# aexoden/snesimage

Hardware: AMD Instinct MI355X
Metric: candidate palettes scored/sec (higher is better)
Workload: dtype f32

## Files before the change

### snesimage_amd/csrc/capi.hip

```cpp
#include "../../include/snesimage_hip.h"
#include "kernels.hpp"
#include "kernels_opt.hpp"
#include "kernels_fast.hpp"
#include "kernels_sparse.hpp"
#include "kernels_sparse2.hpp"
#include "kernels_batch.hpp"
#include "kernels_shared.hpp"
#include "kernels_tile.hpp"
#include "kernels_level.hpp"
#include "kernels_char.hpp"
#include "kernels_char_set.hpp"
#include "kernels_guide.hpp"
#include "kernels_guide_lab.hpp"
#include "kernels_guide_window.hpp"

#include <hip/hip_runtime.h>

#include <atomic>
#include <cmath>
#include <cstdio>
#include <cstdlib>
#include <cstring>
#include <string>
#include <utility>
// ... 124 lines not shown
        bool counters_cleared = false;
        uint32_t h2q_max = 512;
        bool down_tiles = true;
        uint32_t h0_min = 1024;
        bool base_down_side = false;
        uint32_t h0_grid = 8192;
        hipStream_t h0_stream[8] = {}; hipEvent_t ev_scan[8] = {}, ev_h0[8] = {}, ev_hn[8] = {}, ev_vn[8] = {};
        bool v0_aside = true;
        hipEvent_t ev_v0[8] = {};
        bool vn_aside = true;
        uint32_t tiles_grid = 4096;
        uint32_t down1_grid = 32768;
        bool vsplit = true;
        uint32_t scan4_max = 2048;
        uint32_t hgrid = 8192;
        bool dedup = true; uint32_t dedup_min = 1024; int *holder = nullptr; bool holder_dirty = false;
        bool enabled = false, side = true; uint32_t min_n = 1; uint32_t cap = 0, lanes = 0;
        SparseGeom S{};
        float *store = nullptr, *cand_tab = nullptr, *cand_lab = nullptr, *ckf = nullptr, *ckh = nullptr; long long zeros_off = 0; uint32_t *bitmap = nullptr; double *cka = nullptr, *part = nullptr;
        CandMeta *meta = nullptr; unsigned int *items = nullptr; int *item_count = nullptr; long long item_stride = 0; int *order = nullptr, *first = nullptr;
        uint4 *plist = nullptr; int *plist_count = nullptr; bool plist_valid = false;
        hipStream_t base_stream = nullptr; hipEvent_t ev_base_in = nullptr, ev_base_h = nullptr, ev_base_done = nullptr, ev_base_narrow = nullptr;
        uint8_t *dmaps = nullptr, *dmapsC4 = nullptr;
        uint8_t *bmap = nullptr, *bmapC4 = nullptr, *bcand = nullptr; unsigned long long *dpack = nullptr; double *ckd = nullptr; uint32_t slot_ci = 0;
        float *rec_lab = nullptr;
        int base_sp = -1, base_si = -1;
        struct Ahead { uint8_t *bmap = nullptr, *bmapC4 = nullptr, *bcand = nullptr; unsigned long long *dpack = nullptr; double *ckd = nullptr; float *btab = nullptr, *blab = nullptr, *rec_lab = nullptr; int *ok = nullptr;
                       hipEvent_t ev = nullptr; bool on = true, have = false; int sp = -1, si = -1; unsigned long long epoch = 0; } ahead;
    } sp;
    uint8_t *d_cand = nullptr; uint32_t cand_cap = 0;
// ... 361 lines not shown
    return SNES_OK;
}

SparseParams sparse_params(snesimage_ctx *c, uint32_t lane) {
    auto &sp = c->sp;
    SparseParams P{};
    P.G = c->G; P.S = sp.S; P.K = c->K; P.ncol = c->ncol; P.base = (int)(sp.lanes * sp.cap);
    P.pack = c->d_pack; P.packC4 = c->d_packC4; P.packR4 = c->d_packR4; P.plist = sp.plist; P.plist_count = sp.plist_count;
    P.pal_lin = c->d_pal_lin; P.pal_xyb = c->d_pal_xyb; P.cand_tab = sp.cand_tab;
    P.perceptual = c->perceptual ? 1 : 0; P.labpx = c->d_labpx_t; P.cand_lab = sp.cand_lab; P.bitmap = sp.bitmap;
    P.img1C4 = c->d_img1C4; P.mu1R4 = c->d_mu1R4; P.sd1R4 = c->d_sd1R4; P.a1R4 = c->d_a1R4; P.r1R4 = c->d_r1R4;
    P.store = sp.store; P.meta = sp.meta;
    P.items = sp.items + (size_t)lane * sp.item_stride * kItemLists; P.item_count = sp.item_count + (size_t)lane * kItemLists; P.item_stride = sp.item_stride;
    P.ckf = sp.ckf; P.cka = sp.cka; P.part = sp.part; P.first = sp.first; P.ckh = sp.ckh; P.zeros = sp.ckh + sp.zeros_off; P.trash = sp.ckh + sp.zeros_off + 12LL * c->G.W;
    for (P.s_first = 0; P.s_first < c->G.nscales && c->G.sw[P.s_first] >= 64; P.s_first++) {}
    if (c->dither) {
        const uint32_t l = lane < c->nlanes ? lane : 0;
        P.use_maps = 1; P.sub_size = (int)c->sub_size; P.slot_ci = sp.slot_ci; P.subC4 = c->d_subC4; P.tile_pal = c->d_tile_pal;
        P.perceptual = 0; P.labpx = sp.rec_lab;
        P.maps = sp.dmaps + (size_t)l * sp.cap * c->npx; P.mapsC4 = sp.dmapsC4 + (size_t)l * sp.cap * c->npx; P.bmap = sp.bmap; P.bmapC4 = sp.bmapC4;
    }
    return P;
}

static size_t h2_lds(const snesimage_ctx *c) { return sizeof(float) * 3 * (size_t)(c->ncol + 2); }

int32_t sparse_base_pass(snesimage_ctx *c, int sp_idx, int si, uint32_t n_cand) {
    auto &sp = c->sp;
    const Geom &G = c->G;
    if (!sp.plist_valid) {
// ... 474 lines not shown
    if (const char *e = getenv("SNES_DITHER_REC")) c->dither_rec = atoi(e) != 0;
    if (const char *e = getenv("SNES_DITHER4_MAX")) { int v = atoi(e); if (v >= 0) c->dither4_max = (uint32_t)v; }
    if (const char *e = getenv("SNES_DOWN1_GRID")) { int v = atoi(e); if (v >= 64) c->sp.down1_grid = (uint32_t)v; }
    if (const char *e = getenv("SNES_VSPLIT")) c->sp.vsplit = atoi(e) != 0;
    if (const char *e = getenv("SNES_DOWN_TILES")) c->sp.down_tiles = atoi(e) != 0;
    if (const char *e = getenv("SNES_V0_ASIDE")) c->sp.v0_aside = atoi(e) != 0;
    if (const char *e = getenv("SNES_VN_ASIDE")) c->sp.vn_aside = atoi(e) != 0;
    if (const char *e = getenv("SNES_H0_GRID")) { int v = atoi(e); if (v >= 16) c->sp.h0_grid = (uint32_t)v; }
    if (const char *e = getenv("SNES_H0_MIN")) { int v = atoi(e); if (v >= 0) c->sp.h0_min = (uint32_t)v; }
    if (const char *e = getenv("SNES_TILES_GRID")) { int v = atoi(e); if (v >= 64) c->sp.tiles_grid = (uint32_t)v; }
    if (const char *e = getenv("SNES_SCAN4_MAX")) { int v = atoi(e); if (v >= 0) c->sp.scan4_max = (uint32_t)v; }
    if (const char *e = getenv("SNES_H2Q_MAX")) { int v = atoi(e); if (v >= 0) c->sp.h2q_max = (uint32_t)v; }
    if (const char *e = getenv("SNES_HGRID")) { int v = atoi(e); if (v >= 1) c->sp.hgrid = (uint32_t)v; }
    if (const char *e = getenv("SNES_SPARSE_MIN")) { int v = atoi(e); if (v >= 1) c->sp.min_n = (uint32_t)v; }
    if (const char *e = getenv("SNES_DEDUP")) c->sp.dedup = atoi(e) != 0;
    if (const char *e = getenv("SNES_DEDUP_MIN")) { int v = atoi(e); if (v >= 1) c->sp.dedup_min = (uint32_t)v; }
    Geom &G = c->G;
    G.W = (int)w; G.H = (int)h; G.nscales = 0;
    int P2 = 8;
    while (P2 < (int)h) P2 *= 2;
    for (int s = 0; s < kMaxScales; s++) {
        if (s > 0 && (G.sw[s - 1] < 8 || G.th[s - 1] < 8)) break;
        G.sw[s] = (int)w >> s; G.th[s] = s == 0 ? (int)h : (G.th[s - 1] + 1) / 2; G.sh[s] = s == 0 ? (int)h : P2 >> s; G.nscales = s + 1;
    }
    long long off = 0, soff = 0;
    for (int s = 0; s < G.nscales; s++) {
        long long N = (long long)G.sw[s] * G.sh[s];
        G.src_off[s] = soff; soff += 3 * N;
        if (s >= 1) { G.off_xyb[s] = off; off += 3 * N; G.off_xybT[s] = off; off += 3 * N; } else { G.off_xyb[s] = 0; G.off_xybT[s] = 0; }
        G.off_hout[s] = off; off += 9 * N;
// ... 553 lines not shown
```

### snesimage_amd/csrc/kernels.hpp

```cpp
#pragma once
#include "color.hpp"

namespace snes {

constexpr int kMaxScales = SSIM2_NUM_SCALES;
constexpr int kBlurRadius = 5;

SNES_HD long long idx_c4(int x, int y, int H) { return ((long long)(x >> 2) * H + y) * 4 + (x & 3); }
SNES_HD long long idx_r4(int x, int y, int W) { return ((long long)(y >> 2) * W + x) * 4 + (y & 3); }
SNES_HD long long idx_xt4(int x, int y, int H) { return ((((long long)(x >> 6) * (H >> 2)) + (y >> 2)) << 8) + ((x & 63) << 2) + (y & 3); }

struct BlurK {
    float n2[3];
    float d1[3];
};

struct Geom {
    int W, H, nscales;
    int sw[kMaxScales], sh[kMaxScales];
    int th[kMaxScales];
    long long off_xyb[kMaxScales], off_xybT[kMaxScales], off_hout[kMaxScales];
    long long cand_stride;
    long long src_off[kMaxScales];
};

inline unsigned down_grid(const Geom &G) { return (unsigned)((G.W / 32) * ((2 * G.sh[1] + 31) / 32)); }
SNES_HD int down_odd_row(const Geom &G, int s, int y) { return 2 * y + 1 < G.th[s - 1] ? 2 * y + 1 : 2 * y; }

__device__ __constant__ double kSsim2Weight[108] = SSIM2_WEIGHTS;

__global__ void k_palette_tables(const uint8_t *__restrict__ colors , int ncol, const float *__restrict__ eotf ,
                                 uint32_t *__restrict__ pal_rgb8, float *__restrict__ pal_lin, float *__restrict__ pal_xyb) {
    int i = blockIdx.x * blockDim.x + threadIdx.x;
    if (i >= ncol + 2) return;
    uint32_t rgb8 = 0;
    if (i < ncol) rgb8 = rgb5_to_rgb8(colors[3 * i], colors[3 * i + 1], colors[3 * i + 2]);
    float r = eotf[rgb8 & 0xff], g = eotf[(rgb8 >> 8) & 0xff], b = eotf[(rgb8 >> 16) & 0xff];
    float X, Y, B;
    linear_to_positive_xyb(r, g, b, X, Y, B);
    pal_rgb8[i] = rgb8;
    pal_lin[3 * i] = r; pal_lin[3 * i + 1] = g; pal_lin[3 * i + 2] = b;
    pal_xyb[3 * i] = X; pal_xyb[3 * i + 1] = Y; pal_xyb[3 * i + 2] = B;
}

// ... 321 lines not shown
                                                       float *__restrict__ lin0, float *__restrict__ img1, float *__restrict__ img1T) {
    int px = blockIdx.x * blockDim.x + threadIdx.x;
    if (px >= W * H) return;
    int x = px % W, y = px / W;
    uint32_t o = reinterpret_cast<const uint32_t *>(orig)[px];
    float r = eotf[o & 0xff], g = eotf[(o >> 8) & 0xff], b = eotf[(o >> 16) & 0xff];
    size_t n = (size_t)W * H;
    lin0[px] = r; lin0[n + px] = g; lin0[2 * n + px] = b;
    float X, Y, B;
    linear_to_positive_xyb(r, g, b, X, Y, B);
    img1[px] = X; img1[n + px] = Y; img1[2 * n + px] = B;
    size_t pt = (size_t)x * H + y;
    img1T[pt] = X; img1T[n + pt] = Y; img1T[2 * n + pt] = B;
}

__device__ __forceinline__ void maps_accumulate(double (&acc)[6], float m1, float sd1, float a1, double r1, float m2, float v22, float v12, float i2) {
    const float mu22 = m2 * m2, mu12 = m1 * m2;
    const float mu_diff = m1 - m2;
    const float num_m = fmaf(mu_diff, -mu_diff, 1.0f);
    const float num_s = fmaf(2.0f, v12 - mu12, SSIM2_C2);
    const float denom_s = sd1 + (v22 - mu22) + SSIM2_C2;
    double d = 1.0 - (double)((num_m * num_s) / denom_s);
    d = d > 0.0 ? d : 0.0;
    acc[0] += d;
    const double dd = d * d;
    acc[1] += dd * dd;
    const double d1 = ((double)fabsf(i2 - m2) - (double)a1) * r1;
    const double art = d1 > 0.0 ? d1 : 0.0;
    const double det = (-d1) > 0.0 ? (-d1) : 0.0;
    acc[2] += art;
    const double a2 = art * art;
    acc[3] += a2 * a2;
    acc[4] += det;
    const double l2 = det * det;
    acc[5] += l2 * l2;
}
__device__ __forceinline__ float source_sd1(float mu1, float sigma11) { const float mu11 = mu1 * mu1; return sigma11 - mu11; }
__device__ __forceinline__ float source_a1(float img1, float mu1) { return fabsf(img1 - mu1); }
__device__ __forceinline__ double source_r1(float a1) { return 1.0 / (1.0 + (double)a1); }
__global__ __launch_bounds__(256) void k_src_pad_rows(Geom G, float *__restrict__ sd1, double *__restrict__ r1) {
    const int s = (int)blockIdx.y;
    if (s >= G.nscales) return;
    const int W = G.sw[s], pad = G.sh[s] - G.th[s];
    const int n = 3 * W * pad;
    for (int i = (int)(blockIdx.x * blockDim.x + threadIdx.x); i < n; i += (int)(gridDim.x * blockDim.x)) {
        const int c = i / (W * pad), rem = i - c * (W * pad);
        const size_t idx = (size_t)G.src_off[s] + (size_t)c * W * G.sh[s] + (size_t)G.th[s] * W + rem;
        sd1[idx] = __builtin_nanf("");
        r1[idx] = 0.0;
    }
// ... 318 lines not shown
```

### snesimage_amd/csrc/kernels_batch.hpp

```cpp
#pragma once
#include "kernels_sparse2.hpp"

namespace snes {

struct BatchArgs {
    SparseParams Pc, Pb;
    PrepParams prep;
    unsigned long long key; const uint8_t *colors_in; uint8_t *colors; uint8_t *cand; const float *eotf; float *cand_tab;
    const double *part; double *errors; double *inc_err; StepResult *last; PaletteTables T;
    int method, n, slot, channel, nes, npx;
    const float *lab_eotf; float *cand_lab;
    DitherParams Db, Dc; const unsigned long long *win_pack; const uint8_t *bcolor; float *btab; int *zero; int nzero; uint8_t *map;
    int dead_base;
};

#define SNES_BATCH_IMG if (dead && *dead >= A[0].dead_base) return; const BatchArgs &a = A[blockIdx.z]
struct BatchBlock { int img, x, y; };
__device__ __forceinline__ BatchBlock batch_block() {
    BatchBlock b;
    const int X = (int)gridDim.x, Y = (int)gridDim.y, K = (int)gridDim.z;
    const int per = X * Y, K8 = K & ~7;
    const int L = (int)blockIdx.x + X * ((int)blockIdx.y + Y * (int)blockIdx.z);
    int rem;
    if (L < per * K8) { const int idx = L >> 3; b.img = (L & 7) + 8 * (idx / per); rem = idx % per; }
// ... 30 lines not shown
__global__ __launch_bounds__(256) void kb_sparse_down(const BatchArgs *__restrict__ A, int only_scale, const int *__restrict__ dead) { SNES_BATCH_XCD; sparse_down_body(a.Pc, only_scale, bb.x); }
__global__ __launch_bounds__(256) void kb_sparse_down_tiles(const BatchArgs *__restrict__ A, const int *__restrict__ dead) { SNES_BATCH_XCD; sparse_down_tiles_body<SNES_DOWN_TILES_U>(a.Pc, bb.x, (int)gridDim.x); }
__global__ __launch_bounds__(256) void kb_sparse_down1(const BatchArgs *__restrict__ A, const int *__restrict__ dead) { SNES_BATCH_XCD; sparse_down1_body(a.Pc, bb.x, (int)gridDim.x); }
__global__ void kb_candidate_tables(const BatchArgs *__restrict__ A, const int *__restrict__ dead) { SNES_BATCH_IMG; candidate_tables_body(a.cand, a.n, a.eotf, a.cand_tab); }
__global__ void kb_candidate_lab(const BatchArgs *__restrict__ A, const int *__restrict__ dead) { SNES_BATCH_IMG; candidate_lab_body(a.cand_tab, a.n, a.lab_eotf, a.cand_lab); }
__global__ __launch_bounds__(256) void kb_clear_bitmaps(const BatchArgs *__restrict__ A, const int *__restrict__ dead) {
    SNES_BATCH_IMG;
    const size_t words = (size_t)a.n * (a.npx / 32);
    for (size_t i = (size_t)blockIdx.x * 256 + threadIdx.x; i < words; i += (size_t)gridDim.x * 256) a.Pc.bitmap[i] = 0u;
}
__global__ __launch_bounds__(256) void kb_sparse_scan_lab(const BatchArgs *__restrict__ A, const int *__restrict__ dead) { SNES_BATCH_IMG; sparse_scan_lab_body(a.Pc); }
__global__ __launch_bounds__(64) void kb_sparse_h(const BatchArgs *__restrict__ A, int base, const int *__restrict__ dead) { SNES_BATCH_IMG; sparse_h_body(base ? a.Pb : a.Pc); }
__global__ __launch_bounds__(64) void kb_sparse_h2(const BatchArgs *__restrict__ A, const int *__restrict__ dead) { SNES_BATCH_XCD; sparse_h2_dispatch<false>(a.Pc, bb.y, bb.x, (int)gridDim.x); }
__global__ __launch_bounds__(64) void kb_sparse_h2_base(const BatchArgs *__restrict__ A, const int *__restrict__ dead) { SNES_BATCH_XCD; sparse_h2_dispatch<true>(a.Pb, bb.y, bb.x, (int)gridDim.x); }
__global__ __launch_bounds__(64) void kb_sparse_h2_lists(const BatchArgs *__restrict__ A, const int *__restrict__ dead, int list0) { SNES_BATCH_XCD; sparse_h2_dispatch<false>(a.Pc, list0 + bb.y, bb.x, (int)gridDim.x); }
__global__ __launch_bounds__(256, 5) void kb_sparse_v2_scales(const BatchArgs *__restrict__ A, const int *__restrict__ dead, int s0) { SNES_BATCH_XCD; const int s = s0 + bb.y; if (s < a.Pc.G.nscales && a.Pc.G.sw[s] >= 64) sparse_v2_body<false>(a.Pc, s, bb.x); }
__global__ __launch_bounds__(64) void kb_sparse_h2q(const BatchArgs *__restrict__ A, const int *__restrict__ dead) { SNES_BATCH_XCD; sparse_h2q_dispatch<false>(a.Pc, bb.y, bb.x, (int)gridDim.x); }
__global__ __launch_bounds__(64) void kb_sparse_h2q_base(const BatchArgs *__restrict__ A, const int *__restrict__ dead) { SNES_BATCH_XCD; sparse_h2q_dispatch<true>(a.Pb, bb.y, bb.x, (int)gridDim.x); }
__global__ __launch_bounds__(256, 5) void kb_sparse_v2(const BatchArgs *__restrict__ A, const int *__restrict__ dead) { SNES_BATCH_XCD; if (bb.y < a.Pc.G.nscales && a.Pc.G.sw[bb.y] >= 64) sparse_v2_body<false>(a.Pc, bb.y, bb.x); }
__global__ __launch_bounds__(256) void kb_sparse_v_base(const BatchArgs *__restrict__ A, const int *__restrict__ dead) { SNES_BATCH_XCD; if (bb.y < a.Pb.G.nscales && a.Pb.G.sw[bb.y] >= 64) sparse_v2_body<true>(a.Pb, bb.y, bb.x); }
__global__ __launch_bounds__(128) void kb_sparse_v_base_split(const BatchArgs *__restrict__ A, const int *__restrict__ dead) {
    SNES_BATCH_IMG;
    const int s = (int)blockIdx.y / 3, ch = (int)blockIdx.y - 3 * s;
    if (s < a.Pb.G.nscales && a.Pb.G.sw[s] >= 64 && (int)blockIdx.x < (a.Pb.G.sw[s] >> 6)) sparse_v2_base_split_body(a.Pb, s, ch, (int)blockIdx.x);
}
__global__ __launch_bounds__(256, 1) void kb_sparse_v_base_narrow(const BatchArgs *__restrict__ A, const int *__restrict__ dead) { SNES_BATCH_IMG; sparse_v_base_narrow_dispatch(a.Pb); }
__global__ __launch_bounds__(1024) void kb_sparse_order(const BatchArgs *__restrict__ A, const int *__restrict__ dead) { SNES_BATCH_IMG; sparse_order_body(a.Pc, const_cast<int *>(a.Pc.order)); }
__global__ __launch_bounds__(256, 2) void kb_sparse_v(const BatchArgs *__restrict__ A, const int *__restrict__ dead) { SNES_BATCH_IMG; sparse_v_body<false, 2, 2>(a.Pc, (int)blockIdx.y + a.Pc.s_first); }
__global__ __launch_bounds__(256) void kb_final_score(const BatchArgs *__restrict__ A, const int *__restrict__ dead) { SNES_BATCH_IMG; final_score_wave_body(a.part, a.n, a.Pc.G, a.errors, 1, 0, a.Pc.item_count, (int)kItemLists); }
__global__ __launch_bounds__(256) void kb_commit(const BatchArgs *__restrict__ A, const int *__restrict__ dead) { SNES_BATCH_IMG; commit_body(a.errors, a.n, a.cand, a.colors, a.slot, a.nes, a.inc_err, a.last, a.T); }
__global__ __launch_bounds__(1024) void kb_take_map(const BatchArgs *__restrict__ A, const int *__restrict__ dead) {
    SNES_BATCH_IMG;
    const int k = a.last->best_k;
    if (k < 0) return;
    const uint4 *src = reinterpret_cast<const uint4 *>(a.Pc.maps + (size_t)k * a.npx);
// ... 92 lines not shown
```

### snesimage_amd/csrc/kernels_sparse.hpp

```cpp
#pragma once
#include "kernels.hpp"

namespace snes {

constexpr int kGroupsTotal = 126;

struct CandMeta {
    int ngroups[kMaxScales];
    int xmin;
    int won;
    unsigned char glist[kGroupsTotal + 2];
    short gslot[kGroupsTotal];
    unsigned char gcb[kGroupsTotal];
};
__device__ __forceinline__ int item_k(unsigned int it) { return (int)(it >> 14); }
__device__ __forceinline__ int item_g(unsigned int it) { return (int)((it >> 8) & 63u); }
__device__ __forceinline__ int item_j(unsigned int it) { return (int)((it >> 2) & 63u); }
__device__ __forceinline__ int item_ch(unsigned int it) { return (int)(it & 3u); }
constexpr int kColBuckets = 4;
constexpr int kItemLists = kMaxScales * kColBuckets;

struct SparseGeom {
    long long off_lin[kMaxScales], off_xybC[kMaxScales], off_xybR[kMaxScales], off_hout[kMaxScales];
    long long cand_stride;
// ... 8 lines not shown
    const unsigned long long *pack, *packC4, *packR4;
    const uint4 *plist; const int *plist_count;
    const float *pal_lin, *pal_xyb, *cand_tab;
    int perceptual; const float *labpx, *cand_lab; uint32_t *bitmap;
    const float *img1C4, *mu1R4, *sd1R4, *a1R4; const double *r1R4;
    float *store; CandMeta *meta;
    unsigned int *items; int *item_count; long long item_stride;
    float *ckf; double *cka; double *part; float *ckh;
    const float *zeros;
    float *trash;
    int use_maps, sub_size; uint32_t slot_ci; const uint8_t *maps, *mapsC4, *bmap, *bmapC4, *subC4, *tile_pal;
    int s_first;
    int *first;
    const int *order;
    const int *holder; int list0;
};

__device__ __forceinline__ uint32_t sparse_ci(uint32_t lo, uint32_t thr, uint32_t crgb, uint32_t ncol) {
    return red_mean_key(crgb, lo & 0x00ffffffu) < thr ? ncol : (lo >> 24);
}

__device__ __forceinline__ uint32_t won_bit(const uint32_t *bm, int px) { return (bm[px >> 5] >> (px & 31)) & 1u; }
__device__ __forceinline__ uint32_t maps_ci(const SparseParams &P, const uint8_t *map, bool is_base, int x0, int y0, uint32_t pack_lo) {
    uint32_t ci = pack_lo >> 24;
    if (ci != (uint32_t)P.ncol + 1u) {
        ci = (uint32_t)P.tile_pal[(x0 >> 3) + (y0 >> 3) * (P.G.W >> 3)] * (uint32_t)P.sub_size + map[y0 * P.G.W + x0];
        if (!is_base && ci == P.slot_ci) ci = (uint32_t)P.ncol;
    }
    return ci;
}
// ... 1179 lines not shown
```

### snesimage_amd/csrc/kernels_sparse2.hpp

```cpp
#pragma once
#include "kernels_sparse.hpp"
#include "kernels_fast.hpp"

namespace snes {

#define SNES_HSTEP(SUM, A, B, OUT)                                                   \
    {                                                                                \
        float o1_ = (SUM) * n2_0, o3_ = (SUM) * n2_1, o5_ = (SUM) * n2_2;            \
        o1_ = fmaf(-1.0f, B[0], o1_); o3_ = fmaf(-1.0f, B[1], o3_); o5_ = fmaf(-1.0f, B[2], o5_); \
        o1_ = fmaf(mp_0, A[0], o1_); o3_ = fmaf(mp_1, A[1], o3_); o5_ = fmaf(mp_2, A[2], o5_);    \
        B[0] = o1_; B[1] = o3_; B[2] = o5_;                                          \
        OUT = o1_ + o3_ + o5_;                                                       \
    }
#define SNES_VSTEP(SUM, A, B, OUT)                                                   \
    {                                                                                \
        float o1_ = fmaf(A[0], d1_0, B[0]), o3_ = fmaf(A[1], d1_1, B[1]), o5_ = fmaf(A[2], d1_2, B[2]); \
        o1_ = fmaf((SUM), n2_0, -o1_); o3_ = fmaf((SUM), n2_1, -o3_); o5_ = fmaf((SUM), n2_2, -o5_);    \
        B[0] = o1_; B[1] = o3_; B[2] = o5_;                                          \
        OUT = o1_ + o3_ + o5_;                                                       \
    }

struct H2Shared {
    __attribute__((aligned(16))) float out[16 * (4 * 32 + 4)];
    long long hbase[16], xbase[16];
// ... 314 lines not shown
typedef unsigned int u32x4 __attribute__((ext_vector_type(4)));
__device__ __forceinline__ rsrc_t make_rsrc(const void *p) {
    const unsigned long long a = (unsigned long long)p;
    const unsigned long long u = ((unsigned long long)(uint32_t)__builtin_amdgcn_readfirstlane((int)(a >> 32)) << 32) | (uint32_t)__builtin_amdgcn_readfirstlane((int)a);
    return __builtin_amdgcn_make_buffer_rsrc(reinterpret_cast<void *>(u), 0, 0x7fffffff, 0x00020000);
}
__device__ __forceinline__ float4 buf_ld4(rsrc_t r, uint32_t voff, uint32_t soff) {
    const u32x4 v = __builtin_amdgcn_raw_buffer_load_b128(r, (int)voff, (int)soff, 0);
    return make_float4(__uint_as_float(v.x), __uint_as_float(v.y), __uint_as_float(v.z), __uint_as_float(v.w));
}
__device__ __forceinline__ double2 buf_ld2d(rsrc_t r, uint32_t voff, uint32_t soff) {
    const u32x4 v = __builtin_amdgcn_raw_buffer_load_b128(r, (int)voff, (int)soff, 0);
    return make_double2(__hiloint2double((int)v.y, (int)v.x), __hiloint2double((int)v.w, (int)v.z));
}

template <bool BASE>
__device__ __forceinline__ void sparse_v2_body(const SparseParams &P, const int s, const int bx) {
    __shared__ short s_slot[4][64];
    __shared__ __attribute__((aligned(16))) unsigned char s_raw[(2 + 3) * 3 * 256 * sizeof(float2)];
    double (*red)[6] = reinterpret_cast<double (*)[6]>(s_raw);
    static_assert(sizeof(s_raw) >= 256 * 6 * sizeof(double), "reduction scratch must fit the tail ring");
    const Geom &G = P.G;
    const int W = uni(G.sw[s]), H = uni(G.sh[s]), H4 = H >> 2;
    const int t = threadIdx.x, lane = t & 63;
    const int wv = uni(t >> 6);
    const int wpp = W >> 6, ppw = 4 / wpp;
    const int npairs = BASE ? 3 : P.ncand * 3;
    if (bx * ppw >= npairs) return;
    const int ql = wv / wpp, xw = (wv - ql * wpp) << 6;
    const int pair_raw = bx * ppw + ql;
    const bool active = pair_raw < npairs;
    const int pair = active ? pair_raw : 0;
    const int ch = BASE ? pair : pair / P.ncand, ci = BASE ? 0 : pair - ch * P.ncand;
    const int k = BASE ? P.base : uni(P.k0 + (P.order ? P.order[ci] : ci));
    const CandMeta *M = P.meta + k;
    int gs;
// ... 28 lines not shown
    float *ck_f = P.ckf + P.S.off_ckf[s] + ((size_t)ch * (H4 + 2)) * 18 * W + xw + lane;
    double *ck_a = P.cka + P.S.off_cka[s] + ((size_t)ch * (H4 + 2)) * 6 * W + xw + lane;
    if (BASE) {
#pragma unroll
        for (int p = 0; p < 3; p++)
#pragma unroll
            for (int q = 0; q < 3; q++) { sa[p][q] = 0.0f; sb[p][q] = 0.0f; }
#pragma unroll
        for (int q = 0; q < 6; q++) acc[q] = 0.0;
    } else {
        const float *cf = P.ckf + P.S.off_ckf[s] + ((size_t)ch * (H4 + 2) + gs) * 18 * W + xw;
        const double *ca = P.cka + P.S.off_cka[s] + ((size_t)ch * (H4 + 2) + gs) * 6 * W + xw;
#pragma unroll
        for (int p = 0; p < 3; p++)
#pragma unroll
            for (int q = 0; q < 3; q++) { sa[p][q] = ld_at<float>(cf + (size_t)(p * 6 + q) * W, l4); sb[p][q] = ld_at<float>(cf + (size_t)(p * 6 + 3 + q) * W, l4); }
#pragma unroll
        for (int q = 0; q < 6; q++) acc[q] = ld_at<double>(ca + (size_t)q * W, l8);
    }
#define SNES_HLOAD(GG, DST)                                                                                                   \
    {                                                                                                                         \
        const int gg_ = (GG);                                                                                                 \
        const bool below_ = gg_ >= H4;                                                                                        \
        const int sl_ = uni((int)s_slot[wv][below_ ? 0 : gg_]);                                                               \
        const rsrc_t r_ = below_ ? h_zero : (sl_ >= 0 ? h_own : h_b);                                                         \
        const uint32_t so_ = below_ ? 0u : (uint32_t)(sl_ >= 0 ? sl_ : gg_) * 9u * W16;                                       \
        DST[0] = buf_ld4(r_, l16, so_); DST[1] = buf_ld4(r_, l16, so_ + W16); DST[2] = buf_ld4(r_, l16, so_ + 2u * W16);      \
    }
    const float4 zero4 = make_float4(0.f, 0.f, 0.f, 0.f);
    float2 *ring_xy = reinterpret_cast<float2 *>(s_raw) + t;
    float2 *ring_zw = reinterpret_cast<float2 *>(s_raw + 2 * 3 * 256 * sizeof(float2)) + t;
    float4 bufA[3], bufB[3];
    float4 t1[3] = {zero4, zero4, zero4}, t2[3] = {zero4, zero4, zero4}, t3[3] = {zero4, zero4, zero4};
#pragma unroll
    for (int p = 0; p < 3; p++) { bufA[p] = zero4; bufB[p] = zero4; }
    if (gs <= H4) {
        if (gs < H4) SNES_HLOAD(gs, bufA)
        if (gs - 1 >= 0) SNES_HLOAD(gs - 1, t1)
        if (gs - 2 >= 0) SNES_HLOAD(gs - 2, t2)
        if (gs - 3 >= 0) SNES_HLOAD(gs - 3, t3)
    }
#pragma unroll
    for (int p = 0; p < 3; p++) {
        const float4 g1 = t1[p], g2 = t2[p], g3 = t3[p];
        ring_xy[(1 * 3 + p) * 256] = make_float2(g1.x, g1.y); ring_zw[(2 * 3 + p) * 256] = make_float2(g1.z, g1.w);
        ring_xy[(0 * 3 + p) * 256] = make_float2(g2.x, g2.y); ring_zw[(1 * 3 + p) * 256] = make_float2(g2.z, g2.w);
        ring_zw[(0 * 3 + p) * 256] = make_float2(g3.z, g3.w);
    }
    int r2 = 0, r3 = 0;
#define SNES_V2GROUP(CUR, NXT)                                                                                                \
    {                                                                                                                         \
        if (BASE && active) {                                                                                   \
            _Pragma("unroll") for (int p = 0; p < 3; p++)                                                                     \
                _Pragma("unroll") for (int q = 0; q < 3; q++) { ck_f[(size_t)(p * 6 + q) * W] = sa[p][q]; ck_f[(size_t)(p * 6 + 3 + q) * W] = sb[p][q]; } \
            _Pragma("unroll") for (int q = 0; q < 6; q++) ck_a[(size_t)q * W] = acc[q];                                       \
            ck_f += (size_t)18 * W; ck_a += (size_t)6 * W;                                                                    \
        }                                                                                                                     \
        SNES_HLOAD(g + 1, NXT)                                                                                                \
                \
        float4 c_m1, c_sd1, c_a1, c_x;                                                                                        \
        double2 c_ra, c_rb;                                                                                                   \
        {                                                                                                                     \
            const int gm = g >= 1 ? g - 1 : 0;                                                                                \
            const uint32_t go = (uint32_t)gm * W16;                                                                           \
            c_m1 = buf_ld4(m1_b, l16, go); c_sd1 = buf_ld4(sd1_b, l16, go); c_a1 = buf_ld4(a1_b, l16, go);                    \
            c_ra = buf_ld2d(r1_b, l32, 2u * go); c_rb = buf_ld2d(r1_b, l32 + 16u, 2u * go);                                   \
            const int sl = uni((int)s_slot[wv][gm]);                                                                          \
            c_x = buf_ld4(sl >= 0 ? x_own : x_b, l16, (uint32_t)(sl >= 0 ? sl : gm) * 3u * W16);                              \
        }                                                                                                                     \
        float outp[3][4];                                                                                                     \
        _Pragma("unroll") for (int p = 0; p < 3; p++) {                                                                       \
            float2 *pz = ring_zw + (r3 * 3 + p) * 256, *px = ring_xy + (r2 * 3 + p) * 256;                                    \
            const float2 tz = *pz, tx = *px;                                       \
            *pz = make_float2(CUR[p].z, CUR[p].w);                                                                            \
            *px = make_float2(CUR[p].x, CUR[p].y);                                                                            \
            SNES_VSTEP(tz.x + CUR[p].x, sa[p], sb[p], outp[p][0])                                                             \
            SNES_VSTEP(tz.y + CUR[p].y, sb[p], sa[p], outp[p][1])                                                             \
            SNES_VSTEP(tx.x + CUR[p].z, sa[p], sb[p], outp[p][2])                                                             \
            SNES_VSTEP(tx.y + CUR[p].w, sb[p], sa[p], outp[p][3])                                                             \
        }                                                                                                                     \
          \
        asm volatile("" : "+v"(c_a1.x), "+v"(c_a1.y), "+v"(c_a1.z), "+v"(c_a1.w));                                            \
        if (g >= 1) {                                                                                                         \
            const float m1v[4] = {c_m1.x, c_m1.y, c_m1.z, c_m1.w}, sd1v[4] = {c_sd1.x, c_sd1.y, c_sd1.z, c_sd1.w};              \
            const float a1v[4] = {c_a1.x, c_a1.y, c_a1.z, c_a1.w}, i2v[4] = {c_x.x, c_x.y, c_x.z, c_x.w};                     \
            const double r1v[4] = {c_ra.x, c_ra.y, c_rb.x, c_rb.y};                                                           \
            _Pragma("unroll") for (int q = 0; q < 4; q++)                                                                     \
                maps_accumulate(acc, m1v[q], sd1v[q], a1v[q], r1v[q], outp[0][q], outp[1][q], outp[2][q], i2v[q]);            \
        }                                                                                                                     \
        r2 ^= 1; r3 = r3 == 2 ? 0 : r3 + 1;                                                                                   \
    }
    for (int g = gs; g <= H4; g++) {
        SNES_V2GROUP(bufA, bufB)
        g++;
        if (g > H4) break;
        SNES_V2GROUP(bufB, bufA)
    }
#undef SNES_V2GROUP
#undef SNES_HLOAD
    if (BASE && active) {
#pragma unroll
        for (int q = 0; q < 6; q++) ck_a[(size_t)q * W] = acc[q];
    }
    __syncthreads();
#pragma unroll
    for (int q = 0; q < 6; q++) red[t][q] = active ? acc[q] : 0.0;
    __syncthreads();
    const int xp = t & (W - 1);
    for (int stride = W >> 1; stride > 0; stride >>= 1) {
        if (xp < stride) {
#pragma unroll
            for (int q = 0; q < 6; q++) red[t][q] += red[t + stride][q];
        }
        __syncthreads();
    }
    if (xp == 0 && active) {
        double *o = P.part + (((size_t)k * G.nscales + s) * 3 + ch) * 6;
#pragma unroll
        for (int q = 0; q < 6; q++) o[q] = red[t][q];
    }
}
__device__ __forceinline__ void lds_barrier() { asm volatile("s_waitcnt lgkmcnt(0)\n\ts_barrier" ::: "memory"); }
__device__ __forceinline__ void sparse_v2_base_split_body(const SparseParams &P, const int s, const int ch, const int cb) {
    __shared__ __attribute__((aligned(16))) float s_x[2][3][64][4];
    const Geom &G = P.G;
    const int W = uni(G.sw[s]), H = uni(G.sh[s]), H4 = H >> 2;
    const int lane = threadIdx.x & 63;
    const bool is_r = uni((int)(threadIdx.x >> 6)) == 0;
    const int xw = cb << 6;
    const size_t ns = (size_t)W * H;
    const float *store_b = P.store + (size_t)P.base * P.S.cand_stride;
    const uint32_t l16 = (uint32_t)lane << 4, l32 = (uint32_t)lane << 5;
    const uint32_t W16 = (uint32_t)W * 16u;
    const float4 zero4 = make_float4(0.f, 0.f, 0.f, 0.f);
    if (is_r) {
// ... 82 lines not shown
#undef SNES_HSTEP
#undef SNES_VSTEP

template <bool BASE>
__device__ __forceinline__ void sparse_h2_dispatch(const SparseParams &P, const int list, const int bx, const int gx) {
    const int s = list / kColBuckets;
    if (s >= P.G.nscales || P.G.sw[s] < 64 || (list % kColBuckets) >= (P.G.sw[s] >> 6)) return;
    __shared__ H2Shared sh;
    if (s == 0) sparse_h2_body<true, BASE>(P, list, bx, gx, sh); else sparse_h2_body<false, BASE>(P, list, bx, gx, sh);
}
__global__ __launch_bounds__(64) void k_sparse_h2(SparseParams P) { sparse_h2_dispatch<false>(P, (int)blockIdx.y, (int)blockIdx.x, (int)gridDim.x); }
__global__ __launch_bounds__(64) void k_sparse_h2_from(SparseParams P, int list0) { sparse_h2_dispatch<false>(P, list0 + (int)blockIdx.y, (int)blockIdx.x, (int)gridDim.x); }
__global__ __launch_bounds__(64) void k_sparse_h2q(SparseParams P) { sparse_h2q_dispatch<false>(P, (int)blockIdx.y, (int)blockIdx.x, (int)gridDim.x); }
__global__ __launch_bounds__(64) void k_sparse_h2q_base(SparseParams P) { sparse_h2q_dispatch<true>(P, (int)blockIdx.y, (int)blockIdx.x, (int)gridDim.x); }
__global__ __launch_bounds__(64) void k_sparse_h2_base(SparseParams P) { sparse_h2_dispatch<true>(P, (int)blockIdx.y, (int)blockIdx.x, (int)gridDim.x); }
__global__ __launch_bounds__(256, 5) void k_sparse_v2(SparseParams P) { if ((int)blockIdx.y < P.G.nscales && P.G.sw[blockIdx.y] >= 64) sparse_v2_body<false>(P, (int)blockIdx.y, (int)blockIdx.x); }
__global__ __launch_bounds__(256, 5) void k_sparse_v2_from(SparseParams P, int s0) { const int s = s0 + (int)blockIdx.y; if (s < P.G.nscales && P.G.sw[s] >= 64) sparse_v2_body<false>(P, s, (int)blockIdx.x); }
__global__ __launch_bounds__(128) void k_sparse_v2_base_split(SparseParams P) { const int s = (int)blockIdx.z; if (s < P.G.nscales && P.G.sw[s] >= 64 && (int)blockIdx.x < (P.G.sw[s] >> 6)) sparse_v2_base_split_body(P, s, (int)blockIdx.y, (int)blockIdx.x); }
__global__ __launch_bounds__(256) void k_sparse_v2_base(SparseParams P) { if ((int)blockIdx.y < P.G.nscales && P.G.sw[blockIdx.y] >= 64) sparse_v2_body<true>(P, (int)blockIdx.y, (int)blockIdx.x); }
__device__ __forceinline__ void sparse_v_base_narrow_dispatch(const SparseParams &P) { const int s = (int)blockIdx.y + P.s_first; if (s < P.G.nscales) sparse_v_body<false, 0, 1>(P, s); }
__global__ __launch_bounds__(256, 1) void k_sparse_v_base_narrow(SparseParams P) { sparse_v_base_narrow_dispatch(P); }

}
```

Measured before the change: 2.923 million.

## Skip SSIM2 sum terms whose final weight is zero in sparse vertical pass

Builds compile-time masks from the SSIM2 weight table that record which of the six per-scale/channel accumulators actually carry nonzero weight. The candidate vertical-pass kernel picks a specialized template instance per block, so it skips loads, ring updates and accumulation for the unused SSIM or edge terms and writes zeros for them. It also reads the kernel parameters directly from the kernarg segment to avoid copying them. In exchange it generates several template variants, which grows code size and adds a per-block dispatch branch. An env var restores the full sums.

Result: faster. 3.233 million (median of 6 runs) (+10.6%).

```diff
diff --git a/snesimage_amd/csrc/capi.hip b/snesimage_amd/csrc/capi.hip
--- a/snesimage_amd/csrc/capi.hip
+++ b/snesimage_amd/csrc/capi.hip
@@ -162,6 +162,7 @@
         bool vsplit = true;
         uint32_t scan4_max = 2048;
         uint32_t hgrid = 8192;
+        bool weight_mask = true;
         bool dedup = true; uint32_t dedup_min = 1024; int *holder = nullptr; bool holder_dirty = false;
         bool enabled = false, side = true; uint32_t min_n = 1; uint32_t cap = 0, lanes = 0;
         SparseGeom S{};
@@ -553,6 +554,7 @@
     P.items = sp.items + (size_t)lane * sp.item_stride * kItemLists; P.item_count = sp.item_count + (size_t)lane * kItemLists; P.item_stride = sp.item_stride;
     P.ckf = sp.ckf; P.cka = sp.cka; P.part = sp.part; P.first = sp.first; P.ckh = sp.ckh; P.zeros = sp.ckh + sp.zeros_off; P.trash = sp.ckh + sp.zeros_off + 12LL * c->G.W;
     for (P.s_first = 0; P.s_first < c->G.nscales && c->G.sw[P.s_first] >= 64; P.s_first++) {}
+    P.full_sums = sp.weight_mask ? 0 : 1;
     if (c->dither) {
         const uint32_t l = lane < c->nlanes ? lane : 0;
         P.use_maps = 1; P.sub_size = (int)c->sub_size; P.slot_ci = sp.slot_ci; P.subC4 = c->d_subC4; P.tile_pal = c->d_tile_pal;
@@ -1057,6 +1059,7 @@
     if (const char *e = getenv("SNES_HGRID")) { int v = atoi(e); if (v >= 1) c->sp.hgrid = (uint32_t)v; }
     if (const char *e = getenv("SNES_SPARSE_MIN")) { int v = atoi(e); if (v >= 1) c->sp.min_n = (uint32_t)v; }
     if (const char *e = getenv("SNES_DEDUP")) c->sp.dedup = atoi(e) != 0;
+    if (const char *e = getenv("SNES_WEIGHT_MASK")) c->sp.weight_mask = atoi(e) != 0;
     if (const char *e = getenv("SNES_DEDUP_MIN")) { int v = atoi(e); if (v >= 1) c->sp.dedup_min = (uint32_t)v; }
     Geom &G = c->G;
     G.W = (int)w; G.H = (int)h; G.nscales = 0;
diff --git a/snesimage_amd/csrc/kernels.hpp b/snesimage_amd/csrc/kernels.hpp
--- a/snesimage_amd/csrc/kernels.hpp
+++ b/snesimage_amd/csrc/kernels.hpp
@@ -28,6 +28,50 @@
 SNES_HD int down_odd_row(const Geom &G, int s, int y) { return 2 * y + 1 < G.th[s - 1] ? 2 * y + 1 : 2 * y; }
 
 __device__ __constant__ double kSsim2Weight[108] = SSIM2_WEIGHTS;
+
+constexpr int kSumAll = 0x3f, kSumSsim = 0x03, kSumEdge = 0x3c;
+struct SumMaskTable { unsigned char m[kMaxScales + 1][3][kMaxScales]; };
+constexpr double kSsim2WeightHost[108] = SSIM2_WEIGHTS;
+constexpr SumMaskTable make_sum_masks() {
+    SumMaskTable t{};
+    const int acc_of[6] = {0, 2, 4, 1, 3, 5};
+    for (int ns = 1; ns <= kMaxScales; ns++)
+        for (int ch = 0; ch < 3; ch++)
+            for (int s = 0; s < ns; s++) {
+                int m = 0;
+                for (int e = 0; e < 6; e++) if (kSsim2WeightHost[(ch * ns + s) * 6 + e] != 0.0) m |= 1 << acc_of[e];
+                t.m[ns][ch][s] = (unsigned char)m;
+            }
+    return t;
+}
+constexpr SumMaskTable kSumMasksHost = make_sum_masks();
+__device__ __constant__ SumMaskTable kSumMasks = make_sum_masks();
+constexpr int kSumClasses = 10;
+struct SumClassTable { unsigned char m[kSumClasses]; };
+constexpr SumClassTable make_sum_classes() {
+    SumClassTable t{};
+    int n = 0;
+    for (int ch = 0; ch < 3; ch++)
+        for (int s = 0; s < 3 && s < kMaxScales; s++) {
+            const unsigned char m = kSumMasksHost.m[kMaxScales][ch][s];
+            bool seen = false;
+            for (int i = 0; i < n; i++) seen = seen || t.m[i] == m;
+            if (!seen) t.m[n++] = m;
+        }
+    for (; n < kSumClasses; n++) t.m[n] = (unsigned char)kSumAll;
+    return t;
+}
+constexpr SumClassTable kSumClassesHost = make_sum_classes();
+__device__ __constant__ SumClassTable kSumClassTab = make_sum_classes();
+constexpr bool sum_class_is_first(int i) { for (int j = 0; j < i; j++) if (kSumClassesHost.m[j] == kSumClassesHost.m[i]) return false; return true; }
+__device__ __forceinline__ int sum_class(const int need) {
+    int best = kSumClasses - 1, bits = 7;
+    for (int i = 0; i < kSumClasses; i++) {
+        const int m = kSumClassTab.m[i];
+        if ((m & need) == need && __builtin_popcount(m) < bits) { best = i; bits = __builtin_popcount(m); }
+    }
+    return best;
+}
 
 __global__ void k_palette_tables(const uint8_t *__restrict__ colors , int ncol, const float *__restrict__ eotf ,
                                  uint32_t *__restrict__ pal_rgb8, float *__restrict__ pal_lin, float *__restrict__ pal_xyb) {
@@ -379,26 +423,41 @@
     img1T[pt] = X; img1T[n + pt] = Y; img1T[2 * n + pt] = B;
 }
 
+template <int MASK = kSumAll>
 __device__ __forceinline__ void maps_accumulate(double (&acc)[6], float m1, float sd1, float a1, double r1, float m2, float v22, float v12, float i2) {
-    const float mu22 = m2 * m2, mu12 = m1 * m2;
-    const float mu_diff = m1 - m2;
-    const float num_m = fmaf(mu_diff, -mu_diff, 1.0f);
-    const float num_s = fmaf(2.0f, v12 - mu12, SSIM2_C2);
-    const float denom_s = sd1 + (v22 - mu22) + SSIM2_C2;
-    double d = 1.0 - (double)((num_m * num_s) / denom_s);
-    d = d > 0.0 ? d : 0.0;
-    acc[0] += d;
-    const double dd = d * d;
-    acc[1] += dd * dd;
-    const double d1 = ((double)fabsf(i2 - m2) - (double)a1) * r1;
-    const double art = d1 > 0.0 ? d1 : 0.0;
-    const double det = (-d1) > 0.0 ? (-d1) : 0.0;
-    acc[2] += art;
-    const double a2 = art * art;
-    acc[3] += a2 * a2;
-    acc[4] += det;
-    const double l2 = det * det;
-    acc[5] += l2 * l2;
+    if (MASK & kSumSsim) {
+        const float mu22 = m2 * m2, mu12 = m1 * m2;
+        const float mu_diff = m1 - m2;
+        const float num_m = fmaf(mu_diff, -mu_diff, 1.0f);
+        const float num_s = fmaf(2.0f, v12 - mu12, SSIM2_C2);
+        const float denom_s = sd1 + (v22 - mu22) + SSIM2_C2;
+        double d = 1.0 - (double)((num_m * num_s) / denom_s);
+        d = d > 0.0 ? d : 0.0;
+        if (MASK & 1) acc[0] += d;
+        if (MASK & 2) {
+            const double dd = d * d;
+            acc[1] += dd * dd;
+        }
+    }
+    if (MASK & kSumEdge) {
+        const double d1 = ((double)fabsf(i2 - m2) - (double)a1) * r1;
+        if (MASK & 0x0c) {
+            const double art = d1 > 0.0 ? d1 : 0.0;
+            if (MASK & 4) acc[2] += art;
+            if (MASK & 8) {
+                const double a2 = art * art;
+                acc[3] += a2 * a2;
+            }
+        }
+        if (MASK & 0x30) {
+            const double det = (-d1) > 0.0 ? (-d1) : 0.0;
+            if (MASK & 0x10) acc[4] += det;
+            if (MASK & 0x20) {
+                const double l2 = det * det;
+                acc[5] += l2 * l2;
+            }
+        }
+    }
 }
 __device__ __forceinline__ float source_sd1(float mu1, float sigma11) { const float mu11 = mu1 * mu1; return sigma11 - mu11; }
 __device__ __forceinline__ float source_a1(float img1, float mu1) { return fabsf(img1 - mu1); }
diff --git a/snesimage_amd/csrc/kernels_batch.hpp b/snesimage_amd/csrc/kernels_batch.hpp
--- a/snesimage_amd/csrc/kernels_batch.hpp
+++ b/snesimage_amd/csrc/kernels_batch.hpp
@@ -68,11 +68,11 @@
 __global__ __launch_bounds__(64) void kb_sparse_h2(const BatchArgs *__restrict__ A, const int *__restrict__ dead) { SNES_BATCH_XCD; sparse_h2_dispatch<false>(a.Pc, bb.y, bb.x, (int)gridDim.x); }
 __global__ __launch_bounds__(64) void kb_sparse_h2_base(const BatchArgs *__restrict__ A, const int *__restrict__ dead) { SNES_BATCH_XCD; sparse_h2_dispatch<true>(a.Pb, bb.y, bb.x, (int)gridDim.x); }
 __global__ __launch_bounds__(64) void kb_sparse_h2_lists(const BatchArgs *__restrict__ A, const int *__restrict__ dead, int list0) { SNES_BATCH_XCD; sparse_h2_dispatch<false>(a.Pc, list0 + bb.y, bb.x, (int)gridDim.x); }
-__global__ __launch_bounds__(256, 5) void kb_sparse_v2_scales(const BatchArgs *__restrict__ A, const int *__restrict__ dead, int s0) { SNES_BATCH_XCD; const int s = s0 + bb.y; if (s < a.Pc.G.nscales && a.Pc.G.sw[s] >= 64) sparse_v2_body<false>(a.Pc, s, bb.x); }
+__global__ __launch_bounds__(256, 5) void kb_sparse_v2_scales(const BatchArgs *__restrict__ A, const int *__restrict__ dead, int s0) { SNES_BATCH_XCD; const int s = s0 + bb.y; if (s < a.Pc.G.nscales && a.Pc.G.sw[s] >= 64) sparse_v2_cand(a.Pc, s, bb.x); }
 __global__ __launch_bounds__(64) void kb_sparse_h2q(const BatchArgs *__restrict__ A, const int *__restrict__ dead) { SNES_BATCH_XCD; sparse_h2q_dispatch<false>(a.Pc, bb.y, bb.x, (int)gridDim.x); }
 __global__ __launch_bounds__(64) void kb_sparse_h2q_base(const BatchArgs *__restrict__ A, const int *__restrict__ dead) { SNES_BATCH_XCD; sparse_h2q_dispatch<true>(a.Pb, bb.y, bb.x, (int)gridDim.x); }
-__global__ __launch_bounds__(256, 5) void kb_sparse_v2(const BatchArgs *__restrict__ A, const int *__restrict__ dead) { SNES_BATCH_XCD; if (bb.y < a.Pc.G.nscales && a.Pc.G.sw[bb.y] >= 64) sparse_v2_body<false>(a.Pc, bb.y, bb.x); }
-__global__ __launch_bounds__(256) void kb_sparse_v_base(const BatchArgs *__restrict__ A, const int *__restrict__ dead) { SNES_BATCH_XCD; if (bb.y < a.Pb.G.nscales && a.Pb.G.sw[bb.y] >= 64) sparse_v2_body<true>(a.Pb, bb.y, bb.x); }
+__global__ __launch_bounds__(256, 5) void kb_sparse_v2(const BatchArgs *__restrict__ A, const int *__restrict__ dead) { SNES_BATCH_XCD; if (bb.y < a.Pc.G.nscales && a.Pc.G.sw[bb.y] >= 64) sparse_v2_cand(a.Pc, bb.y, bb.x); }
+__global__ __launch_bounds__(256) void kb_sparse_v_base(const BatchArgs *__restrict__ A, const int *__restrict__ dead) { SNES_BATCH_XCD; if (bb.y < a.Pb.G.nscales && a.Pb.G.sw[bb.y] >= 64) sparse_v2_base(a.Pb, bb.y, bb.x); }
 __global__ __launch_bounds__(128) void kb_sparse_v_base_split(const BatchArgs *__restrict__ A, const int *__restrict__ dead) {
     SNES_BATCH_IMG;
     const int s = (int)blockIdx.y / 3, ch = (int)blockIdx.y - 3 * s;
diff --git a/snesimage_amd/csrc/kernels_sparse.hpp b/snesimage_amd/csrc/kernels_sparse.hpp
--- a/snesimage_amd/csrc/kernels_sparse.hpp
+++ b/snesimage_amd/csrc/kernels_sparse.hpp
@@ -46,6 +46,7 @@
     int *first;
     const int *order;
     const int *holder; int list0;
+    int full_sums;
 };
 
 __device__ __forceinline__ uint32_t sparse_ci(uint32_t lo, uint32_t thr, uint32_t crgb, uint32_t ncol) {
diff --git a/snesimage_amd/csrc/kernels_sparse2.hpp b/snesimage_amd/csrc/kernels_sparse2.hpp
--- a/snesimage_amd/csrc/kernels_sparse2.hpp
+++ b/snesimage_amd/csrc/kernels_sparse2.hpp
@@ -352,12 +352,19 @@
     return make_double2(__hiloint2double((int)v.y, (int)v.x), __hiloint2double((int)v.w, (int)v.z));
 }
 
-template <bool BASE>
-__device__ __forceinline__ void sparse_v2_body(const SparseParams &P, const int s, const int bx) {
-    __shared__ short s_slot[4][64];
-    __shared__ __attribute__((aligned(16))) unsigned char s_raw[(2 + 3) * 3 * 256 * sizeof(float2)];
+struct V2Shared {
+    short slot[4][64];
+    __attribute__((aligned(16))) unsigned char raw[(2 + 3) * 3 * 256 * sizeof(float2)];
+};
+template <bool BASE, int MASK>
+__device__ __forceinline__ void sparse_v2_body(const SparseParams &P, const int s, const int bx, V2Shared &sh) {
+    static_assert(!BASE || MASK == kSumAll, "B's sweep leaves full records");
+    constexpr bool SS = (MASK & kSumSsim) != 0, ED = (MASK & kSumEdge) != 0;
+    constexpr int NPL = SS ? 3 : 1;
+    short (*s_slot)[64] = sh.slot;
+    unsigned char *const s_raw = sh.raw;
     double (*red)[6] = reinterpret_cast<double (*)[6]>(s_raw);
-    static_assert(sizeof(s_raw) >= 256 * 6 * sizeof(double), "reduction scratch must fit the tail ring");
+    static_assert(sizeof(sh.raw) >= 256 * 6 * sizeof(double), "reduction scratch must fit the tail ring");
     const Geom &G = P.G;
     const int W = uni(G.sw[s]), H = uni(G.sh[s]), H4 = H >> 2;
     const int t = threadIdx.x, lane = t & 63;
@@ -416,9 +423,12 @@
 #pragma unroll
         for (int p = 0; p < 3; p++)
 #pragma unroll
-            for (int q = 0; q < 3; q++) { sa[p][q] = ld_at<float>(cf + (size_t)(p * 6 + q) * W, l4); sb[p][q] = ld_at<float>(cf + (size_t)(p * 6 + 3 + q) * W, l4); }
-#pragma unroll
-        for (int q = 0; q < 6; q++) acc[q] = ld_at<double>(ca + (size_t)q * W, l8);
+            for (int q = 0; q < 3; q++) {
+                sa[p][q] = p < NPL ? ld_at<float>(cf + (size_t)(p * 6 + q) * W, l4) : 0.0f;
+                sb[p][q] = p < NPL ? ld_at<float>(cf + (size_t)(p * 6 + 3 + q) * W, l4) : 0.0f;
+            }
+#pragma unroll
+        for (int q = 0; q < 6; q++) acc[q] = ((MASK >> q) & 1) ? ld_at<double>(ca + (size_t)q * W, l8) : 0.0;
     }
 #define SNES_HLOAD(GG, DST)                                                                                                   \
     {                                                                                                                         \
@@ -427,7 +437,8 @@
         const int sl_ = uni((int)s_slot[wv][below_ ? 0 : gg_]);                                                               \
         const rsrc_t r_ = below_ ? h_zero : (sl_ >= 0 ? h_own : h_b);                                                         \
         const uint32_t so_ = below_ ? 0u : (uint32_t)(sl_ >= 0 ? sl_ : gg_) * 9u * W16;                                       \
-        DST[0] = buf_ld4(r_, l16, so_); DST[1] = buf_ld4(r_, l16, so_ + W16); DST[2] = buf_ld4(r_, l16, so_ + 2u * W16);      \
+        DST[0] = buf_ld4(r_, l16, so_);                                                                                       \
+        if (SS) { DST[1] = buf_ld4(r_, l16, so_ + W16); DST[2] = buf_ld4(r_, l16, so_ + 2u * W16); }                          \
     }
     const float4 zero4 = make_float4(0.f, 0.f, 0.f, 0.f);
     float2 *ring_xy = reinterpret_cast<float2 *>(s_raw) + t;
@@ -443,7 +454,7 @@
         if (gs - 3 >= 0) SNES_HLOAD(gs - 3, t3)
     }
 #pragma unroll
-    for (int p = 0; p < 3; p++) {
+    for (int p = 0; p < NPL; p++) {
         const float4 g1 = t1[p], g2 = t2[p], g3 = t3[p];
         ring_xy[(1 * 3 + p) * 256] = make_float2(g1.x, g1.y); ring_zw[(2 * 3 + p) * 256] = make_float2(g1.z, g1.w);
         ring_xy[(0 * 3 + p) * 256] = make_float2(g2.x, g2.y); ring_zw[(1 * 3 + p) * 256] = make_float2(g2.z, g2.w);
@@ -460,18 +471,21 @@
         }                                                                                                                     \
         SNES_HLOAD(g + 1, NXT)                                                                                                \
                 \
-        float4 c_m1, c_sd1, c_a1, c_x;                                                                                        \
-        double2 c_ra, c_rb;                                                                                                   \
+        float4 c_m1 = zero4, c_sd1 = zero4, c_a1 = zero4, c_x = zero4;                                                        \
+        double2 c_ra = make_double2(0.0, 0.0), c_rb = c_ra;                                                                   \
         {                                                                                                                     \
             const int gm = g >= 1 ? g - 1 : 0;                                                                                \
             const uint32_t go = (uint32_t)gm * W16;                                                                           \
-            c_m1 = buf_ld4(m1_b, l16, go); c_sd1 = buf_ld4(sd1_b, l16, go); c_a1 = buf_ld4(a1_b, l16, go);                    \
-            c_ra = buf_ld2d(r1_b, l32, 2u * go); c_rb = buf_ld2d(r1_b, l32 + 16u, 2u * go);                                   \
-            const int sl = uni((int)s_slot[wv][gm]);                                                                          \
-            c_x = buf_ld4(sl >= 0 ? x_own : x_b, l16, (uint32_t)(sl >= 0 ? sl : gm) * 3u * W16);                              \
+            if (SS) { c_m1 = buf_ld4(m1_b, l16, go); c_sd1 = buf_ld4(sd1_b, l16, go); }                                       \
+            if (ED) {                                                                                                         \
+                c_a1 = buf_ld4(a1_b, l16, go);                                                                                \
+                c_ra = buf_ld2d(r1_b, l32, 2u * go); c_rb = buf_ld2d(r1_b, l32 + 16u, 2u * go);                               \
+                const int sl = uni((int)s_slot[wv][gm]);                                                                      \
+                c_x = buf_ld4(sl >= 0 ? x_own : x_b, l16, (uint32_t)(sl >= 0 ? sl : gm) * 3u * W16);                          \
+            }                                                                                                                 \
         }                                                                                                                     \
-        float outp[3][4];                                                                                                     \
-        _Pragma("unroll") for (int p = 0; p < 3; p++) {                                                                       \
+        float outp[3][4] = {};                                                                                                \
+        _Pragma("unroll") for (int p = 0; p < NPL; p++) {                                                                     \
             float2 *pz = ring_zw + (r3 * 3 + p) * 256, *px = ring_xy + (r2 * 3 + p) * 256;                                    \
             const float2 tz = *pz, tx = *px;                                       \
             *pz = make_float2(CUR[p].z, CUR[p].w);                                                                            \
@@ -482,13 +496,13 @@
             SNES_VSTEP(tx.y + CUR[p].w, sb[p], sa[p], outp[p][3])                                                             \
         }                                                                                                                     \
           \
-        asm volatile("" : "+v"(c_a1.x), "+v"(c_a1.y), "+v"(c_a1.z), "+v"(c_a1.w));                                            \
+        if (ED) asm volatile("" : "+v"(c_a1.x), "+v"(c_a1.y), "+v"(c_a1.z), "+v"(c_a1.w));                                    \
         if (g >= 1) {                                                                                                         \
             const float m1v[4] = {c_m1.x, c_m1.y, c_m1.z, c_m1.w}, sd1v[4] = {c_sd1.x, c_sd1.y, c_sd1.z, c_sd1.w};              \
             const float a1v[4] = {c_a1.x, c_a1.y, c_a1.z, c_a1.w}, i2v[4] = {c_x.x, c_x.y, c_x.z, c_x.w};                     \
             const double r1v[4] = {c_ra.x, c_ra.y, c_rb.x, c_rb.y};                                                           \
             _Pragma("unroll") for (int q = 0; q < 4; q++)                                                                     \
-                maps_accumulate(acc, m1v[q], sd1v[q], a1v[q], r1v[q], outp[0][q], outp[1][q], outp[2][q], i2v[q]);            \
+                maps_accumulate<MASK>(acc, m1v[q], sd1v[q], a1v[q], r1v[q], outp[0][q], outp[1][q], outp[2][q], i2v[q]);      \
         }                                                                                                                     \
         r2 ^= 1; r3 = r3 == 2 ? 0 : r3 + 1;                                                                                   \
     }
@@ -506,21 +520,43 @@
     }
     __syncthreads();
 #pragma unroll
-    for (int q = 0; q < 6; q++) red[t][q] = active ? acc[q] : 0.0;
+    for (int q = 0; q < 6; q++) if ((MASK >> q) & 1) red[t][q] = active ? acc[q] : 0.0;
     __syncthreads();
     const int xp = t & (W - 1);
     for (int stride = W >> 1; stride > 0; stride >>= 1) {
         if (xp < stride) {
 #pragma unroll
-            for (int q = 0; q < 6; q++) red[t][q] += red[t + stride][q];
+            for (int q = 0; q < 6; q++) if ((MASK >> q) & 1) red[t][q] += red[t + stride][q];
         }
         __syncthreads();
     }
     if (xp == 0 && active) {
         double *o = P.part + (((size_t)k * G.nscales + s) * 3 + ch) * 6;
 #pragma unroll
-        for (int q = 0; q < 6; q++) o[q] = red[t][q];
-    }
+        for (int q = 0; q < 6; q++) o[q] = ((MASK >> q) & 1) ? red[t][q] : 0.0;
+    }
+}
+__device__ __forceinline__ void sparse_v2_base(const SparseParams &P, const int s, const int bx) {
+    __shared__ V2Shared sh;
+    sparse_v2_body<true, kSumAll>(P, s, bx, sh);
+}
+template <int I>
+__device__ __forceinline__ void sparse_v2_class(const SparseParams &P, const int s, const int bx, V2Shared &sh, const int cls) {
+    constexpr bool first = sum_class_is_first(I);
+    if (first && cls == I) sparse_v2_body<false, kSumClassesHost.m[I]>(P, s, bx, sh);
+    else if constexpr (I + 1 < kSumClasses) sparse_v2_class<I + 1>(P, s, bx, sh, cls);
+}
+__device__ __forceinline__ void sparse_v2_cand(const SparseParams &P, const int s, const int bx) {
+    __shared__ V2Shared sh;
+    const int ppw = 4 / (P.G.sw[s] >> 6), npairs = P.ncand * 3;
+    if (bx * ppw >= npairs) return;
+    int need = kSumAll;
+    if (!P.full_sums) {
+        const int c0 = (bx * ppw) / P.ncand, c1 = min(bx * ppw + ppw - 1, npairs - 1) / P.ncand;
+        need = 0;
+        for (int c = c0; c <= c1; c++) need |= kSumMasks.m[P.G.nscales][c][s];
+    }
+    sparse_v2_class<0>(P, s, bx, sh, uni(sum_class(need)));
 }
 __device__ __forceinline__ void lds_barrier() { asm volatile("s_waitcnt lgkmcnt(0)\n\ts_barrier" ::: "memory"); }
 __device__ __forceinline__ void sparse_v2_base_split_body(const SparseParams &P, const int s, const int ch, const int cb) {
@@ -633,10 +669,11 @@
 __global__ __launch_bounds__(64) void k_sparse_h2q(SparseParams P) { sparse_h2q_dispatch<false>(P, (int)blockIdx.y, (int)blockIdx.x, (int)gridDim.x); }
 __global__ __launch_bounds__(64) void k_sparse_h2q_base(SparseParams P) { sparse_h2q_dispatch<true>(P, (int)blockIdx.y, (int)blockIdx.x, (int)gridDim.x); }
 __global__ __launch_bounds__(64) void k_sparse_h2_base(SparseParams P) { sparse_h2_dispatch<true>(P, (int)blockIdx.y, (int)blockIdx.x, (int)gridDim.x); }
-__global__ __launch_bounds__(256, 5) void k_sparse_v2(SparseParams P) { if ((int)blockIdx.y < P.G.nscales && P.G.sw[blockIdx.y] >= 64) sparse_v2_body<false>(P, (int)blockIdx.y, (int)blockIdx.x); }
-__global__ __launch_bounds__(256, 5) void k_sparse_v2_from(SparseParams P, int s0) { const int s = s0 + (int)blockIdx.y; if (s < P.G.nscales && P.G.sw[s] >= 64) sparse_v2_body<false>(P, s, (int)blockIdx.x); }
+__device__ __forceinline__ const SparseParams &kernarg_params() { return *(const SparseParams *)__builtin_amdgcn_kernarg_segment_ptr(); }
+__global__ __launch_bounds__(256, 5) void k_sparse_v2(SparseParams) { const SparseParams &P = kernarg_params(); if ((int)blockIdx.y < P.G.nscales && P.G.sw[blockIdx.y] >= 64) sparse_v2_cand(P, (int)blockIdx.y, (int)blockIdx.x); }
+__global__ __launch_bounds__(256, 5) void k_sparse_v2_from(SparseParams, int s0) { const SparseParams &P = kernarg_params(); const int s = s0 + (int)blockIdx.y; if (s < P.G.nscales && P.G.sw[s] >= 64) sparse_v2_cand(P, s, (int)blockIdx.x); }
 __global__ __launch_bounds__(128) void k_sparse_v2_base_split(SparseParams P) { const int s = (int)blockIdx.z; if (s < P.G.nscales && P.G.sw[s] >= 64 && (int)blockIdx.x < (P.G.sw[s] >> 6)) sparse_v2_base_split_body(P, s, (int)blockIdx.y, (int)blockIdx.x); }
-__global__ __launch_bounds__(256) void k_sparse_v2_base(SparseParams P) { if ((int)blockIdx.y < P.G.nscales && P.G.sw[blockIdx.y] >= 64) sparse_v2_body<true>(P, (int)blockIdx.y, (int)blockIdx.x); }
+__global__ __launch_bounds__(256) void k_sparse_v2_base(SparseParams P) { if ((int)blockIdx.y < P.G.nscales && P.G.sw[blockIdx.y] >= 64) sparse_v2_base(P, (int)blockIdx.y, (int)blockIdx.x); }
 __device__ __forceinline__ void sparse_v_base_narrow_dispatch(const SparseParams &P) { const int s = (int)blockIdx.y + P.s_first; if (s < P.G.nscales) sparse_v_body<false, 0, 1>(P, s); }
 __global__ __launch_bounds__(256, 1) void k_sparse_v_base_narrow(SparseParams P) { sparse_v_base_narrow_dispatch(P); }
 
```
